# xcompact3d/x3d2

Measured on AMD Instinct MI355X. Metric: DoF*steps/s (whole node), TGV 512^3 per GPU, full fractional step, higher is better.
Workload: dtype f64; 1 GPU; TGV 512x512x512 all-periodic, Re=1600, dt=1e-3, RK3 (3 substeps/step), compact6/classic schemes, rocFFT Poisson (configs[2]); per_gpu=512^3, driver=fused, parallelism=domain decomposition 1x1x1, decomposition=yslabs, decomposition_requested=auto, poisson_z_first=228

## Files before the change

### include/x3d2_hip.h

```cpp
#ifndef X3D2_HIP_H
#define X3D2_HIP_H

#include <stddef.h>

#ifdef X3D_SINGLE_PREC
typedef float x3d_real;
#else
typedef double x3d_real;
#endif

#ifdef __cplusplus
extern "C" {
#endif

enum { X3D_DIR_X = 1, X3D_DIR_Y = 2, X3D_DIR_Z = 3, X3D_DIR_C = 4 };
enum { X3D_BC_PERIODIC = 0, X3D_BC_NEUMANN = 1, X3D_BC_DIRICHLET = 2, X3D_BC_HALO = -1 };
enum { X3D_X_FACE = 1100, X3D_Y_FACE = 1010, X3D_Z_FACE = 110 };
#define X3D_N_HALO 4

typedef struct x3d_backend x3d_backend;
typedef struct x3d_tdsops x3d_tdsops;
typedef struct x3d_poisson x3d_poisson;

const char *x3d_last_error(void);
// ... 188 lines not shown
                       const x3d_real *az, const x3d_real *bz);
int x3d_poisson_destroy(x3d_poisson *p);
int x3d_poisson_fft_forward(x3d_poisson *p, const x3d_real *f_in);
int x3d_poisson_postprocess_000(x3d_poisson *p);
int x3d_poisson_fft_backward(x3d_poisson *p, x3d_real *f_out);
int x3d_poisson_solve_000(x3d_poisson *p, x3d_real *f);
int x3d_poisson_enforce_periodicity_y(x3d_poisson *p, x3d_real *f_out, const x3d_real *f_in);
int x3d_poisson_undo_periodicity_y(x3d_poisson *p, x3d_real *f_out, const x3d_real *f_in);
int x3d_poisson_set_stretching(x3d_poisson *p, int sym, const x3d_real *a0, const x3d_real *a1);
int x3d_poisson_postprocess_010(x3d_poisson *p);
int x3d_poisson_solve_010(x3d_poisson *p, x3d_real *f, x3d_real *temp);
int x3d_poisson_solve_010_rows(x3d_poisson *p, x3d_real *f);
int x3d_transpose_xy(x3d_backend *b_src, x3d_backend *b_dst, x3d_real *dst, const x3d_real *src, int nx, int ny, int nz);
int x3d_transpose_xyz_zxy(x3d_backend *b_src, x3d_backend *b_dst, x3d_real *dst, const x3d_real *src, int nx, int ny, int nz);
int x3d_transpose_zxy_xyz(x3d_backend *b_src, x3d_backend *b_dst, x3d_real *dst, const x3d_real *src, int nx, int ny, int nz);
int x3d_poisson_enforce_periodicity_z(x3d_poisson *p, x3d_real *f_out, const x3d_real *f_in);
int x3d_poisson_undo_periodicity_z(x3d_poisson *p, x3d_real *f_out, const x3d_real *f_in);
int x3d_poisson_postprocess_011(x3d_poisson *p);
int x3d_poisson_get_spectral(x3d_poisson *p, x3d_real *host_interleaved);
int x3d_poisson_set_spectral(x3d_poisson *p, const x3d_real *host_interleaved);

typedef struct x3d_sfft x3d_sfft;
int x3d_sfft_create(x3d_backend *b, x3d_sfft **out, const int nglob[3], int pz, int rz);
int x3d_sfft_destroy(x3d_sfft *p);
int x3d_sfft_sizes(const x3d_sfft *p, long out[4]);
int x3d_sfft_set_waves(x3d_sfft *p, const x3d_real *waves, const x3d_real *ax, const x3d_real *bx, const x3d_real *ay,
                       const x3d_real *by, const x3d_real *az, const x3d_real *bz);
int x3d_sfft_forward_local(x3d_sfft *p, const x3d_real *f_in, x3d_real *sendbuf);
int x3d_sfft_fft_z(x3d_sfft *p, x3d_real *recvbuf, int dir);
int x3d_sfft_postprocess_000(x3d_sfft *p, x3d_real *recvbuf);
int x3d_sfft_backward_local(x3d_sfft *p, const x3d_real *recvbuf, x3d_real *f_out);
int x3d_sfft_create_parts(x3d_backend *b, x3d_sfft **out, const int nglob[3], int pz, int rz, int parts);
int x3d_sfft_fft_z_part(x3d_sfft *p, x3d_real *recvbuf, int dir, int part);
int x3d_sfft_postprocess_000_part(x3d_sfft *p, x3d_real *recvbuf, int part);

typedef struct x3d_sfft010 x3d_sfft010;
int x3d_sfft010_create(x3d_backend *b, x3d_sfft010 **out, const int nglob_cell[3], int pz, int rz);
int x3d_sfft010_destroy(x3d_sfft010 *p);
int x3d_sfft010_sizes(const x3d_sfft010 *p, long out[6]);
int x3d_sfft010_create_parts(x3d_backend *b, x3d_sfft010 **out, const int nglob_cell[3], int pz, int rz, int parts);
int x3d_sfft010_fft_z_part(x3d_sfft010 *p, x3d_real *recvbuf, int dir, int part);
int x3d_sfft010_postprocess_010_part(x3d_sfft010 *p, x3d_real *recvbuf, int part);
int x3d_sfft010_set_waves(x3d_sfft010 *p, const x3d_real *waves, const x3d_real *ax, const x3d_real *bx, const x3d_real *ay,
                          const x3d_real *by, const x3d_real *az, const x3d_real *bz);
int x3d_sfft010_set_stretching(x3d_sfft010 *p, int sym, const x3d_real *a0, const x3d_real *a1);
int x3d_sfft010_periodicity_y(x3d_sfft010 *p, x3d_real *f_out, const x3d_real *f_in, int undo);
int x3d_sfft010_forward_local(x3d_sfft010 *p, const x3d_real *f_in, x3d_real *sendbuf);
int x3d_sfft010_fft_z(x3d_sfft010 *p, x3d_real *recvbuf, int dir);
int x3d_sfft010_postprocess_010(x3d_sfft010 *p, x3d_real *recvbuf);
int x3d_sfft010_backward_local(x3d_sfft010 *p, const x3d_real *sendbuf, x3d_real *f_out);

int x3d_poisson_zfirst_ok(x3d_poisson *p, int *ok);
int x3d_tds_pair_zfirst_ok(x3d_backend *b, const x3d_tdsops *ta, const x3d_tdsops *tb, int *ok);
int x3d_poisson_zfirst_middle(x3d_poisson *p);
int x3d_poisson_zfirst_forward(x3d_poisson *p, const x3d_real *f_in);
int x3d_poisson_zfirst_backward(x3d_poisson *p, x3d_real *f_out);
int x3d_poisson_solve_000_zfirst(x3d_poisson *p, x3d_real *f);
int x3d_poisson_set_stretching_zfirst(x3d_poisson *p, int sym, const x3d_real *a0, const x3d_real *a1);
int x3d_poisson_create_proxy(x3d_backend *b, x3d_poisson **out, x3d_real *spectrum, int ny, long px, int (*middle)(void *user),
                             void *user);
int x3d_poisson_solve_010_rows_zfirst(x3d_poisson *p, x3d_real *f);
int x3d_tds_pair_zfirst(x3d_backend *b, x3d_poisson *poisson, int mode, x3d_real *out1, x3d_real *out2, const x3d_real *in1,
                        const x3d_real *in2, const x3d_tdsops *ta, const x3d_tdsops *tb, int *done);

typedef struct x3d_sfftz x3d_sfftz;
int x3d_sfftz_create(x3d_backend *b, x3d_sfftz **out, const int nglob_cell[3], int py, int ry, int parts);
int x3d_sfftz_destroy(x3d_sfftz *p);
int x3d_sfftz_sizes(const x3d_sfftz *p, long out[16]);
int x3d_sfftz_spectrum(const x3d_sfftz *p, x3d_real **c, int *ny, long *px);
int x3d_sfftz_set_waves(x3d_sfftz *p, const x3d_real *rw, const x3d_real *ax, const x3d_real *bx, const x3d_real *ay,
                        const x3d_real *by, const x3d_real *az, const x3d_real *bz);
int x3d_sfftz_tds_pair(x3d_sfftz *p, int mode, x3d_real *out1, x3d_real *out2, const x3d_real *in1, const x3d_real *in2,
                       const x3d_tdsops *ta, const x3d_tdsops *tb, int *done);
int x3d_sfftz_z(x3d_sfftz *p, x3d_real *f, int inverse);
int x3d_sfftz_z_field(x3d_sfftz *p, x3d_real *f, int inverse);
int x3d_sfftz_x_forward(x3d_sfftz *p, x3d_real *sendbuf, int part);
int x3d_sfftz_y_stage(x3d_sfftz *p, x3d_real *recvbuf, int part, int what);
int x3d_sfftz_x_backward(x3d_sfftz *p, const x3d_real *buf, int part);
int x3d_sfftz_tds_pair_rows(x3d_sfftz *p, int mode, x3d_real *out1, x3d_real *out2, const x3d_real *in1, const x3d_real *in2,
                            const x3d_tdsops *ta, const x3d_tdsops *tb, int y0, int nyr, int *done);
int x3d_sfftz_z_rows(x3d_sfftz *p, x3d_real *f, int inverse, int y0, int nyr);
int x3d_sfftz_x_forward_rows(x3d_sfftz *p, x3d_real *sendbuf, int part, int y0, int nyr);
int x3d_sfftz_x_backward_rows(x3d_sfftz *p, const x3d_real *buf, int part, int y0, int nyr);

typedef struct x3d_pfft x3d_pfft;
int x3d_pfft_create(x3d_backend *b, x3d_pfft **out, const int nglob_cell[3], int py, int pz, int ry, int rz);
int x3d_pfft_destroy(x3d_pfft *p);
int x3d_pfft_sizes(const x3d_pfft *p, long out[8]);
int x3d_pfft_set_waves(x3d_pfft *p, const x3d_real *waves_re, const x3d_real *ax, const x3d_real *bx,
                       const x3d_real *ay, const x3d_real *by, const x3d_real *az, const x3d_real *bz);
int x3d_pfft_fwd_x(x3d_pfft *p, const x3d_real *f_in);
int x3d_pfft_bwd_x(x3d_pfft *p, x3d_real *f_out);
int x3d_pfft_fft_y(x3d_pfft *p, int inverse);
int x3d_pfft_fft_z(x3d_pfft *p, int inverse);
int x3d_pfft_pack_xy(x3d_pfft *p, x3d_real *sendbuf);
int x3d_pfft_unpack_xy(x3d_pfft *p, const x3d_real *recvbuf);
int x3d_pfft_pack_yx(x3d_pfft *p, x3d_real *sendbuf);
int x3d_pfft_unpack_yx(x3d_pfft *p, const x3d_real *recvbuf);
int x3d_pfft_pack_yz(x3d_pfft *p, x3d_real *sendbuf);
int x3d_pfft_unpack_yz(x3d_pfft *p, const x3d_real *recvbuf);
int x3d_pfft_pack_zy(x3d_pfft *p, x3d_real *sendbuf);
int x3d_pfft_unpack_zy(x3d_pfft *p, const x3d_real *recvbuf);
int x3d_pfft_transpose_local(x3d_pfft *p, int which);
int x3d_pfft_own_chunk(x3d_pfft *p, const x3d_real *sendbuf, int rank);
int x3d_pfft_postprocess_000(x3d_pfft *p);
int x3d_pfft_create_parts(x3d_backend *b, x3d_pfft **out, const int nglob_cell[3], int py, int pz, int ry, int rz,
// ... 63 lines not shown
```

### x3d2_amd/_lib.py

```python
import ctypes
import os
import subprocess

from .common import X3dError

HERE = os.path.dirname(os.path.abspath(__file__))
SINGLE = os.environ.get("X3D_SINGLE_PREC") == "1"
LIB_PATH = os.path.join(HERE, "libx3d2_hip_sp.so" if SINGLE else "libx3d2_hip.so")
CSRC = os.path.join(HERE, "csrc")

REAL = ctypes.c_float if SINGLE else ctypes.c_double
NP_REAL = "float32" if SINGLE else "float64"
c_double_p = ctypes.POINTER(REAL)
c_int_p = ctypes.POINTER(ctypes.c_int)
VP = ctypes.c_void_p
I, D, SZT = ctypes.c_int, REAL, ctypes.c_size_t


def torch_real():
    import torch
    return torch.float32 if SINGLE else torch.float64

PROTOTYPES = {
    "x3d_last_error": (ctypes.c_char_p, []),
# ... 103 lines not shown
    "x3d_field_set_face_from_field": (I, [VP, VP, VP, c_int_p, D, I, D]),
    "x3d_set_field_data": (I, [VP, VP, c_double_p, c_int_p]),
    "x3d_get_field_data": (I, [VP, c_double_p, VP, c_int_p]),
    "x3d_set_field_data_pitched": (I, [VP, VP, c_double_p, I, I, c_int_p]),
    "x3d_get_field_data_pitched": (I, [VP, c_double_p, VP, I, I, c_int_p]),
    "x3d_poisson_create": (I, [VP, ctypes.POINTER(VP), c_int_p] + [c_double_p] * 7),
    "x3d_poisson_destroy": (I, [VP]),
    "x3d_poisson_fft_forward": (I, [VP, VP]),
    "x3d_poisson_postprocess_000": (I, [VP]),
    "x3d_poisson_fft_backward": (I, [VP, VP]),
    "x3d_poisson_solve_000": (I, [VP, VP]),
    "x3d_poisson_enforce_periodicity_y": (I, [VP, VP, VP]),
    "x3d_poisson_undo_periodicity_y": (I, [VP, VP, VP]),
    "x3d_poisson_set_stretching": (I, [VP, ctypes.c_int, c_double_p, c_double_p]),
    "x3d_sfftz_spectrum": (I, [VP, ctypes.POINTER(VP), c_int_p, ctypes.POINTER(ctypes.c_long)]),
    "x3d_poisson_create_proxy": (I, [VP, ctypes.POINTER(VP), VP, I, ctypes.c_long, VP, VP]),
    "x3d_poisson_set_stretching_zfirst": (I, [VP, ctypes.c_int, c_double_p, c_double_p]),
    "x3d_poisson_postprocess_010": (I, [VP]),
    "x3d_poisson_solve_010": (I, [VP, VP, VP]),
    "x3d_poisson_solve_010_rows": (I, [VP, VP]),
    "x3d_poisson_solve_010_rows_zfirst": (I, [VP, VP]),
    "x3d_poisson_get_spectral": (I, [VP, c_double_p]),
    "x3d_poisson_set_spectral": (I, [VP, c_double_p]),
    "x3d_sfft_create": (I, [VP, ctypes.POINTER(VP), c_int_p, I, I]),
    "x3d_sfft_create_parts": (I, [VP, ctypes.POINTER(VP), c_int_p, I, I, I]),
    "x3d_sfft_fft_z_part": (I, [VP, VP, I, I]),
    "x3d_sfft_postprocess_000_part": (I, [VP, VP, I]),
    "x3d_sfft_destroy": (I, [VP]),
    "x3d_sfft_sizes": (I, [VP, ctypes.POINTER(ctypes.c_long)]),
    "x3d_sfft_set_waves": (I, [VP] + [c_double_p] * 7),
    "x3d_sfft_forward_local": (I, [VP, VP, VP]),
    "x3d_sfft_fft_z": (I, [VP, VP, I]),
    "x3d_sfft_postprocess_000": (I, [VP, VP]),
    "x3d_sfft_backward_local": (I, [VP, VP, VP]),
    "x3d_sfft010_create": (I, [VP, ctypes.POINTER(VP), c_int_p, I, I]),
    "x3d_sfft010_create_parts": (I, [VP, ctypes.POINTER(VP), c_int_p, I, I, I]),
    "x3d_sfft010_fft_z_part": (I, [VP, VP, I, I]),
    "x3d_sfft010_postprocess_010_part": (I, [VP, VP, I]),
    "x3d_sfft010_destroy": (I, [VP]),
    "x3d_sfft010_sizes": (I, [VP, ctypes.POINTER(ctypes.c_long)]),
    "x3d_sfft010_set_waves": (I, [VP] + [c_double_p] * 7),
    "x3d_sfft010_set_stretching": (I, [VP, I, c_double_p, c_double_p]),
    "x3d_sfft010_periodicity_y": (I, [VP, VP, VP, I]),
    "x3d_sfft010_forward_local": (I, [VP, VP, VP]),
    "x3d_sfft010_fft_z": (I, [VP, VP, I]),
    "x3d_sfft010_postprocess_010": (I, [VP, VP]),
    "x3d_sfft010_backward_local": (I, [VP, VP, VP]),
    "x3d_poisson_zfirst_ok": (I, [VP, c_int_p]),
    "x3d_poisson_zfirst_middle": (I, [VP]),
    "x3d_poisson_zfirst_forward": (I, [VP, VP]),
    "x3d_poisson_zfirst_backward": (I, [VP, VP]),
    "x3d_poisson_solve_000_zfirst": (I, [VP, VP]),
    "x3d_tds_pair_zfirst": (I, [VP, VP, I, VP, VP, VP, VP, VP, VP, c_int_p]),
    "x3d_sfftz_create": (I, [VP, ctypes.POINTER(VP), c_int_p, I, I, I]),
    "x3d_sfftz_destroy": (I, [VP]),
    "x3d_sfftz_sizes": (I, [VP, ctypes.POINTER(ctypes.c_long)]),
    "x3d_sfftz_set_waves": (I, [VP] + [c_double_p] * 7),
    "x3d_sfftz_tds_pair": (I, [VP, I, VP, VP, VP, VP, VP, VP, c_int_p]),
    "x3d_sfftz_z": (I, [VP, VP, I]),
    "x3d_sfftz_z_field": (I, [VP, VP, I]),
    "x3d_sfftz_x_forward": (I, [VP, VP, I]),
    "x3d_sfftz_y_stage": (I, [VP, VP, I, I]),
    "x3d_sfftz_x_backward": (I, [VP, VP, I]),
    "x3d_sfftz_tds_pair_rows": (I, [VP, I, VP, VP, VP, VP, VP, VP, I, I, c_int_p]),
    "x3d_sfftz_z_rows": (I, [VP, VP, I, I, I]),
    "x3d_sfftz_x_forward_rows": (I, [VP, VP, I, I, I]),
    "x3d_sfftz_x_backward_rows": (I, [VP, VP, I, I, I]),
    "x3d_pfft_create": (I, [VP, ctypes.POINTER(VP), c_int_p, I, I, I, I]),
    "x3d_pfft_destroy": (I, [VP]),
    "x3d_pfft_sizes": (I, [VP, ctypes.POINTER(ctypes.c_long)]),
    "x3d_pfft_set_waves": (I, [VP] + [c_double_p] * 7),
    "x3d_pfft_fwd_x": (I, [VP, VP]),
    "x3d_pfft_bwd_x": (I, [VP, VP]),
    "x3d_pfft_fft_y": (I, [VP, I]),
    "x3d_pfft_fft_z": (I, [VP, I]),
    "x3d_pfft_pack_xy": (I, [VP, VP]),
    "x3d_pfft_unpack_xy": (I, [VP, VP]),
    "x3d_pfft_pack_yx": (I, [VP, VP]),
    "x3d_pfft_unpack_yx": (I, [VP, VP]),
    "x3d_pfft_pack_yz": (I, [VP, VP]),
    "x3d_pfft_unpack_yz": (I, [VP, VP]),
    "x3d_pfft_pack_zy": (I, [VP, VP]),
    "x3d_pfft_unpack_zy": (I, [VP, VP]),
    "x3d_pfft_transpose_local": (I, [VP, I]),
    "x3d_pfft_own_chunk": (I, [VP, VP, I]),
    "x3d_pfft_postprocess_000": (I, [VP]),
    "x3d_pfft_create_parts": (I, [VP, ctypes.POINTER(VP), c_int_p, I, I, I, I, I]),
    "x3d_pfft_part_layout": (I, [VP, ctypes.POINTER(ctypes.c_long)]),
    "x3d_pfft_fwd_a_part": (I, [VP, VP, VP, I]),
    "x3d_pfft_fwd_b_part": (I, [VP, VP, VP, I]),
    "x3d_pfft_fwd_c_part": (I, [VP, VP, I]),
    "x3d_pfft_bwd_c_part": (I, [VP, VP, I]),
    "x3d_pfft_bwd_b_part": (I, [VP, VP, VP, I]),
    "x3d_pfft_bwd_a_part": (I, [VP, VP, VP, I]),
    "x3d_stats_update_uvw": (I, [VP, VP, VP, VP, ctypes.POINTER(VP), D]),
    "x3d_stats_update_scalar": (I, [VP, VP, VP, VP, D]),
    "x3d_stats_derive": (I, [VP, ctypes.POINTER(VP), ctypes.POINTER(VP)]),
    "x3d_stats_profile_sums": (I, [VP, VP, VP, VP, c_int_p, I, VP]),
    "x3d_stats_profile_accumulate": (I, [VP, VP, VP, ctypes.c_long, D, D]),
    "x3d_ibm_create": (I, [VP, c_double_p, c_int_p, ctypes.POINTER(VP)]),
    "x3d_ibm_destroy": (I, [VP]),
    "x3d_ibm_counts": (I, [VP, ctypes.POINTER(ctypes.c_long)]),
    "x3d_ibm_body": (I, [VP, VP, VP, VP, VP, c_int_p]),
    "x3d_outflow_params": (I, [VP, VP, c_int_p, D, D, ctypes.POINTER(VP)]),
    "x3d_outflow_params_get": (I, [VP, c_double_p]),
    "x3d_cylinder_apply_bc": (I, [VP, VP, VP, VP, VP, VP, VP, c_int_p, VP]),
# ... 51 lines not shown
```

### x3d2_amd/csrc/backend.hip

```cpp
#include <mutex>

#include <algorithm>
#include <vector>

#include "common.h"

#include <unordered_map>
#include <unordered_set>

#include <cmath>

static thread_local char g_err[512] = "";

void x3d_set_error(const char *fmt, ...)
{
    va_list ap;
    va_start(ap, fmt);
    vsnprintf(g_err, sizeof g_err, fmt, ap);
    va_end(ap);
}

extern "C" const char *x3d_last_error(void) { return g_err; }
extern "C" int x3d_abi_version(void) { return 1; }
extern "C" int x3d_real_bytes(void) { return (int)sizeof(real_t); }
// ... 50 lines not shown
    X3D_HIP(hipMalloc(&b->red_buf, sizeof(real_t) * 2 * b->red_cap));
    X3D_HIP(hipHostMalloc(&b->red_host, sizeof(real_t) * 2 * b->red_cap));
    X3D_HIP(hipMalloc(&b->epi_dev, 512));
    b->lds_optin = new std::unordered_set<const void *>();
    X3D_HIP(hipEventCreate(&b->ev0));
    X3D_HIP(hipEventCreate(&b->ev1));
    *out = b;
    return 0;
}

extern "C" int x3d_backend_create_like(x3d_backend **out, const x3d_backend *like, const int dims_vert[3])
{
    X3D_RANGE(__func__);
    X3D_REQUIRE(like, "x3d_backend_create_like: null argument");
    return x3d_backend_create(out, dims_vert, like->device, (void *)like->stream);
}

extern "C" int x3d_backend_destroy(x3d_backend *b)
{
    X3D_RANGE(__func__);
    if (!b) return 0;
    if (b->ipc_maps) {
        auto *v = static_cast<std::vector<void *> *>(b->ipc_maps);
        for (void *p : *v) (void)hipIpcCloseMemHandle(p);
        delete v;
    }
    hipFree(b->send_s); hipFree(b->send_e);
    hipFree(b->scratch[0]); hipFree(b->scratch[1]); hipFree(b->scratch[2]);
    x3d_prof_enable_c(b, 0);
    hipFree(b->red_buf); hipHostFree(b->red_host); hipFree(b->epi_dev);
    if (b->stats_part) hipFree(b->stats_part);
    if (b->bc_params) hipFree(b->bc_params);
    if (b->bc_part) hipFree(b->bc_part);
    hipEventDestroy(b->ev0); hipEventDestroy(b->ev1);
    delete static_cast<std::unordered_set<const void *> *>(b->lds_optin);
    x3d_lazy_destroy(b);
    delete b;
    return 0;
}

int x3d_lds_optin(x3d_backend *b, const void *kernel)
{
    auto *seen = static_cast<std::unordered_set<const void *> *>(b->lds_optin);
    if (seen->count(kernel)) return 0;
    X3D_HIP(hipFuncSetAttribute(kernel, hipFuncAttributeMaxDynamicSharedMemorySize, 160 * 1024));
    seen->insert(kernel);
    return 0;
}

extern "C" long x3d_backend_counter(const x3d_backend *b, int which)
{
    X3D_RANGE(__func__);
    if (!b) return -1;
    return which == 0 ? b->n_tq3 : (which == 1 ? b->n_upd : (which == 2 ? b->n_halo : (which == 3 ? b->n_sync : -1)));
}

extern "C" int x3d_backend_set_stream(x3d_backend *b, void *stream)
{
    X3D_RANGE(__func__);
    X3D_REQUIRE(b, "null backend");
    b->stream = (hipStream_t)stream;
    return 0;
}

extern "C" int x3d_backend_set_comm_reserve(x3d_backend *b, int ncus)
{
    X3D_RANGE(__func__);
    X3D_REQUIRE(b, "null backend");
    X3D_REQUIRE(ncus >= 0 && ncus < X3D_NCU / 2, "x3d_backend_set_comm_reserve: 0 .. %d CUs", X3D_NCU / 2 - 1);
    b->comm_reserve = ncus;
    return 0;
}

extern "C" int x3d_backend_set_ring(x3d_backend *b, int dir, int periodic_over_all_ranks)
{
    X3D_RANGE(__func__);
    X3D_REQUIRE(b && x3d_dir_ok(dir), "x3d_backend_set_ring: null backend or bad direction");
    b->ring[dir] = periodic_over_all_ranks ? 1 : 0;
    return 0;
}

extern "C" size_t x3d_block_elems(const x3d_backend *b) { return b ? b->nblock : 0; }

extern "C" int x3d_padded_dims(const x3d_backend *b, int d[3])
{
    X3D_RANGE(__func__);
    X3D_REQUIRE(b && d, "null argument");
    d[0] = b->nxp; d[1] = b->nyp; d[2] = b->nzp;
    return 0;
}

extern "C" int x3d_device_sync(x3d_backend *b)
{
    X3D_RANGE(__func__);
    if (b) X3D_LAZY_FLUSH(b);
    X3D_LAZY_EAGER(b);
    X3D_REQUIRE(b, "null backend");
    X3D_HIP(hipStreamSynchronize(b->stream));
    return 0;
}

static std::unordered_map<real_t *, void *> g_block_base;
static int g_block_count = 0;
static std::mutex g_block_mutex;

extern "C" int x3d_block_alloc(x3d_backend *b, real_t **out)
{
// ... 840 lines not shown
```

### x3d2_amd/csrc/common.h

```cpp
#pragma once
#include <hip/hip_runtime.h>

#include <cstdarg>
#include <cstdio>
#include <cstring>
#include <vector>

#include "../../include/x3d2_hip.h"

typedef x3d_real real_t;
#ifdef X3D_SINGLE_PREC
typedef float2 real2_t;
#define make_real2 make_float2
#else
typedef double2 real2_t;
#define make_real2 make_double2
#endif
#ifdef X3D_SINGLE_PREC
#define X3D_FFT_R2C HIPFFT_R2C
#define X3D_FFT_C2R HIPFFT_C2R
#define X3D_FFT_C2C HIPFFT_C2C
#define x3d_fftExecR2C hipfftExecR2C
#define x3d_fftExecC2R hipfftExecC2R
#define x3d_fftExecC2C hipfftExecC2C
// ... 43 lines not shown
    __builtin_amdgcn_wave_barrier();
    __builtin_amdgcn_fence(__ATOMIC_ACQUIRE, "wavefront");
}

typedef real_t x3d_d2v __attribute__((ext_vector_type(2)));
__device__ __forceinline__ real2_t ldg_stream(const real2_t *p)
{
    const x3d_d2v v = __builtin_nontemporal_load(reinterpret_cast<const x3d_d2v *>(p));
    return make_real2(v.x, v.y);
}
__device__ __forceinline__ void stg_stream(real2_t *p, real2_t v)
{
    const x3d_d2v w = {v.x, v.y};
    __builtin_nontemporal_store(w, reinterpret_cast<x3d_d2v *>(p));
}

static __device__ __attribute__((used)) float g_vmcnt_sink[32 * 1024];
template <int N>
__device__ __forceinline__ void vmcnt_pad_stores()
{
#pragma unroll
    for (int k = 0; k < N; k++) __builtin_nontemporal_store(0.0f, &g_vmcnt_sink[k * 1024 + (threadIdx.x & 1023)]);
}

__host__ __device__ static inline unsigned long long x3d_mix64(unsigned long long z)
{
    z += 0x9E3779B97F4A7C15ull;
    z = (z ^ (z >> 30)) * 0xBF58476D1CE4E5B9ull;
    z = (z ^ (z >> 27)) * 0x94D049BB133111EBull;
    return z ^ (z >> 31);
}

struct PencilGeom {
    int np;
    int dim0;
    long s0, s1, rs;
};

struct x3d_backend {
    int device;
    hipStream_t stream;
    int nx, ny, nz;
    int ring[4];
    int nxp, nyp, nzp;
    size_t nblock;
    real_t *send_s, *send_e;
    real_t *scratch[3];
    real_t *red_buf;
    real_t *red_host;
    int red_cap;
    long n_upd;
    long n_tq3;
    long n_halo;
    void *epi_dev;
    hipEvent_t ev0, ev1;
    void *ipc_maps;
    struct x3d_prof *prof;
    unsigned prof_mask;
    int pair_yperm;
    void *lds_optin;
    struct x3d_lazy *lazy;
    int comm_reserve;
    double *stats_part;
    long stats_cap;
    real_t *bc_params;
    double *bc_part;
    long n_sync;
};
#define X3D_BC_PARTS 1024
struct TileEpi {
    real_t *y;
    const real_t *base;
    const real_t *x[5];
    real_t c[5];
    int n, ipend, store;
};
#define X3D_NCU 256
static inline int x3d_persistent_blocks(const x3d_backend *b, long want)
{
    const long cap = X3D_NCU - (b->comm_reserve > 0 && b->comm_reserve < X3D_NCU / 2 ? b->comm_reserve : 0);
    return (int)(want > cap ? cap : want);
}

bool x3d_lazy_active(const x3d_backend *b);
void x3d_lazy_destroy(x3d_backend *b);
void x3d_lazy_register(x3d_backend *b, real_t *h);
void x3d_lazy_unregister(x3d_backend *b, real_t *h);
int x3d_lazy_flush_c(x3d_backend *b);
int x3d_lazy_sync_c(x3d_backend *b);
int x3d_lazy_in(x3d_backend *b, const real_t *h, const real_t **out);
int x3d_lazy_out(x3d_backend *b, real_t *h, bool full, real_t **out);
int x3d_lazy_transeq(x3d_backend *b, int dir, real_t *du, real_t *dv, real_t *dw, const real_t *u, const real_t *v,
                     const real_t *w, real_t nu, const x3d_tdsops *t0, const x3d_tdsops *t1, const x3d_tdsops *t2,
                     const x3d_tdsops *t3);
int x3d_lazy_tds(x3d_backend *b, real_t *du, const real_t *u, const x3d_tdsops *t, int dir);
int x3d_lazy_species(x3d_backend *b, int dir, real_t *dspec, const real_t *uvw, const real_t *spec, real_t nu,
                     const x3d_tdsops *t0, const x3d_tdsops *t1, const x3d_tdsops *t2, int accumulate);
int x3d_lazy_copy(x3d_backend *b, real_t *dst, const real_t *src);
int x3d_lazy_sum(x3d_backend *b, real_t *u, const real_t *u_, int dir);
int x3d_lazy_vecadd(x3d_backend *b, real_t a, const real_t *x, real_t bb, real_t *y);
int x3d_lazy_unary(x3d_backend *b, int kind, real_t *f, const real_t *x, real_t a);
int x3d_lazy_fft(x3d_backend *b, int which, void *poisson, real_t *f);
int x3d_lazy_setface(x3d_backend *b, real_t *f, const real_t *f_start, const int dims[3]);
bool x3d_lazy_set_executing(x3d_backend *b, bool on);
struct LazyScope {
    x3d_backend *b;
// ... 140 lines not shown
```

### x3d2_amd/csrc/sfftz.hip

```cpp
#include "zfft_tile.h"

#define SZ_PX 520
#define SZ_MAXPARTS 8

int x3d_fft512_init();
const real2_t *x3d_fft512_twiddles();
int x3d_fft512_peers_yl(x3d_backend *b, real2_t *R, long W, int npeers, const real_t *rw, const real_t *ab, int nx, int ny,
                        int nz, int xs, int xoff, int kz0, int part);
int x3d_ztile_fft_run(x3d_backend *b, real_t *f, const ZfArg &zf, bool fwd, int y0, int nyr);
int x3d_ytile_tds_pair_zf(x3d_backend *b, int mode, real_t *out1, real_t *out2, const real_t *in1, const real_t *in2,
                          const x3d_tdsops *ta, const x3d_tdsops *tb, const ZfArg &zf, bool *done, int y0, int nyr);

struct x3d_sfftz {
    x3d_backend *b;
    int py, ry, xs, xoff, parts;
    int kz0[SZ_MAXPARTS + 1];
    long off[SZ_MAXPARTS + 1];
    real2_t *c;
    real_t *rw;
    real_t *ab;
};

template <bool PACK>
__global__ void __launch_bounds__(512)
// ... 79 lines not shown
    return 0;
}

extern "C" int x3d_sfftz_set_waves(x3d_sfftz *p, const real_t *rw, const real_t *ax, const real_t *bx, const real_t *ay,
                                   const real_t *by, const real_t *az, const real_t *bz)
{
    X3D_RANGE(__func__);
    X3D_REQUIRE(p && rw && ax && bx && ay && by && az && bz, "null argument");
    X3D_HIP(hipMemcpy(p->rw, rw, sizeof(real_t) * 257 * p->xs * 512 * p->py, hipMemcpyHostToDevice));
    real_t *d = p->ab;
    const real_t *src[6] = {ax, bx, ay, by, az, bz};
    const int len[6] = {512, 512, 512 * p->py, 512 * p->py, 512, 512};
    for (int i = 0; i < 6; i++) {
        X3D_HIP(hipMemcpy(d, src[i], sizeof(real_t) * len[i], hipMemcpyHostToDevice));
        d += len[i];
    }
    return 0;
}

static ZfArg zfarg(const x3d_sfftz *p) { return ZfArg{p->c, x3d_fft512_twiddles(), 512, (long)SZ_PX}; }

extern "C" int x3d_sfftz_tds_pair(x3d_sfftz *p, int mode, real_t *out1, real_t *out2, const real_t *in1, const real_t *in2,
                                  const x3d_tdsops *ta, const x3d_tdsops *tb, int *done)
{
    X3D_RANGE(__func__);
    X3D_REQUIRE(p && ta && tb && done, "x3d_sfftz_tds_pair: null argument");
    X3D_REQUIRE(mode == 0 || mode == 1, "x3d_sfftz_tds_pair: mode must be 0 or 1");
    X3D_REQUIRE(mode == 0 ? (in1 && in2) : (out1 && out2 && out1 != out2), "x3d_sfftz_tds_pair: null argument");
    X3D_LAZY_SYNC(p->b);
    X3D_LAZY_EAGER(p->b);
    bool ok = false;
    *done = 0;
    if (int rc = x3d_ytile_tds_pair_zf(p->b, mode, out1, out2, in1, in2, ta, tb, zfarg(p), &ok, 0, -1)) return rc;
    *done = ok ? 1 : 0;
    return 0;
}
extern "C" int x3d_sfftz_tds_pair_rows(x3d_sfftz *p, int mode, real_t *out1, real_t *out2, const real_t *in1,
                                       const real_t *in2, const x3d_tdsops *ta, const x3d_tdsops *tb, int y0, int nyr, int *done)
{
    X3D_RANGE(__func__);
    X3D_REQUIRE(p && ta && tb && done, "x3d_sfftz_tds_pair_rows: null argument");
    X3D_REQUIRE(mode == 0 || mode == 1, "x3d_sfftz_tds_pair_rows: mode must be 0 or 1");
    X3D_REQUIRE(mode == 0 ? (in1 && in2) : (out1 && out2 && out1 != out2), "x3d_sfftz_tds_pair_rows: null argument");
    X3D_REQUIRE(y0 >= 0 && nyr >= 0 && y0 + nyr <= 512, "x3d_sfftz_tds_pair_rows: rows [%d, %d) of 512", y0, y0 + nyr);
    X3D_LAZY_SYNC(p->b);
    X3D_LAZY_EAGER(p->b);
    bool ok = false;
    *done = 0;
    if (int rc = x3d_ytile_tds_pair_zf(p->b, mode, out1, out2, in1, in2, ta, tb, zfarg(p), &ok, y0, nyr)) return rc;
    *done = ok ? 1 : 0;
    return 0;
}

extern "C" int x3d_sfftz_z(x3d_sfftz *p, real_t *f, int inverse)
{
    X3D_RANGE(__func__);
    X3D_REQUIRE(p && f, "null argument");
    X3D_LAZY_SYNC(p->b);
    return x3d_ztile_fft_run(p->b, f, zfarg(p), !inverse, 0, -1);
}
extern "C" int x3d_sfftz_z_field(x3d_sfftz *p, real_t *f, int inverse)
{
    X3D_RANGE(__func__);
    X3D_REQUIRE(p && f, "null argument");
    if (inverse) { X3D_LAZY_OUT(p->b, f, true); }
    else {
        const real_t *fi = f;
        X3D_LAZY_IN(p->b, fi);
        f = const_cast<real_t *>(fi);
    }
    return x3d_ztile_fft_run(p->b, f, zfarg(p), !inverse, 0, -1);
}
extern "C" int x3d_sfftz_z_rows(x3d_sfftz *p, real_t *f, int inverse, int y0, int nyr)
{
    X3D_RANGE(__func__);
    X3D_REQUIRE(p && f, "null argument");
    X3D_REQUIRE(y0 >= 0 && nyr >= 0 && y0 + nyr <= 512, "x3d_sfftz_z_rows: rows [%d, %d) of 512", y0, y0 + nyr);
    X3D_LAZY_SYNC(p->b);
    return x3d_ztile_fft_run(p->b, f, zfarg(p), !inverse, y0, nyr);
}

#define SZ_PART(p, m, name) X3D_REQUIRE((p) && (m) >= 0 && (m) < (p)->parts, name ": part %d of %d", (m), (p) ? (p)->parts : 0)

template <bool PACK>
static int x_xchg(x3d_sfftz *p, real_t *buf, int m, int y0 = 0, int nyr = 512)
{
    const int lds = sizeof(real2_t) * (8 * FP + 256);
    X3D_LDS_OPTIN(p->b, (k_c2c512_x_xchg<PACK>));
    const int kzc = p->kz0[m + 1] - p->kz0[m];
    if (nyr == 0) return 0;
    long blocks = ((long)kzc * nyr + 7) / 8;
    if (blocks > 2048) blocks = 2048;
    ProfScope ps(p->b, X3D_K_FFT, PACK ? 1 : 2);
    hipLaunchKernelGGL((k_c2c512_x_xchg<PACK>), dim3((unsigned)blocks), dim3(512), lds, p->b->stream, p->c,
                       (real2_t *)buf + p->off[m], x3d_fft512_twiddles(), p->kz0[m], kzc, p->xs, y0, nyr);
    X3D_HIP(hipGetLastError());
    return 0;
}
extern "C" int x3d_sfftz_x_forward(x3d_sfftz *p, real_t *sendbuf, int m)
{
    X3D_RANGE(__func__);
    SZ_PART(p, m, "x3d_sfftz_x_forward");
    X3D_REQUIRE(sendbuf, "null argument");
    return x_xchg<true>(p, sendbuf, m);
}
extern "C" int x3d_sfftz_y_stage(x3d_sfftz *p, real_t *recvbuf, int m, int what)
// ... 37 lines not shown
```

### x3d2_amd/csrc/xscan.hip

```cpp
#include "common.h"


int npmax_of(const x3d_backend *b);

#include "xscan_core.h"
#include "zfft_tile.h"


template <bool ACC>
__device__ __forceinline__ void store_rows_q8(real_t *__restrict__ orow, int lane, const real_t (&r)[8],
                                              real_t scale)
{
    const int j = lane & 3;
    real_t a0 = r[0], a1 = r[1], b0 = r[2], b1 = r[3], c0 = r[4], c1 = r[5], d0 = r[6], d1 = r[7];
    rotl_pairs(a0, a1, b0, b1, c0, c1, d0, d1, j);
    b0 = dpp_quad(b0, 1); b1 = dpp_quad(b1, 1);
    c0 = dpp_quad(c0, 2); c1 = dpp_quad(c1, 2);
    d0 = dpp_quad(d0, 3); d1 = dpp_quad(d1, 3);
    rotl_pairs(a0, a1, b0, b1, c0, c1, d0, d1, j);
    real2_t *__restrict__ o2 = reinterpret_cast<real2_t *>(orow + (lane & ~3) * 8) + j;
    real2_t v0, v1, v2, v3;
    if (ACC) {
        v0 = o2[0]; v1 = o2[4]; v2 = o2[8]; v3 = o2[12];
        v0.x += scale * a0; v0.y += scale * a1;
// ... 1558 lines not shown
        return t->tab.bulk_only && t->n_tds == 64 * Q && t->tab.n_rhs == t->n_tds;
    };
    if (!fast(ta) || !fast(tb) || (dir == X3D_DIR_Y ? b->ny : b->nz) != 64 * Q || b->nx % 16 != 0) return 0;
    if (dir == X3D_DIR_Z) { const char *e = getenv("X3D_NO_ZTILE"); if (e && e[0] == '1') return 0; }
    const bool narrow = stencil_narrow(ta) && stencil_narrow(tb);
    static int uni_on = -1;
    if (uni_on < 0) { const char *e = getenv("X3D_NO_UNIFORM"); uni_on = (e && e[0] == '1') ? 0 : 1; }
    const bool uni = uni_on && ta->uniform && tb->uniform;
    const bool circ = narrow && uni && circ_env_on() && (halo ? pair_halo_circ(b, dir, ta, tb) : (ta->circ_ok && tb->circ_ok));
    const size_t lds = sizeof(real_t) * ((size_t)(circ ? 0 : (mode == 2 ? 1 : 2) * LT_N(Q) * 64) + 16 * (64 * Q + 4) + (halo ? 128 + 64 : 0));
    if (lds > 160 * 1024) return 0;
    const long pxy = (long)b->nxp * b->nyp;
    const int ntx = b->nx / 16;
    int tile0, ntiles;
    tile_range(b, dir, other0, nother, ntx, &tile0, &ntiles);
    const int permn = b->pair_yperm;
    if (permn > 0 && (dir != X3D_DIR_Z || mode == 2 || tile0 != 0 || (ntiles > 0 && ntiles != ntx * b->ny))) return 0;
    if (ntiles <= 0) { *done = true; return 0; }
    const long rstride = dir == X3D_DIR_Y ? (long)b->nxp : pxy, ostride = dir == X3D_DIR_Y ? pxy : (long)b->nxp;
    if (128 * rstride * X3D_RB >= (1L << 32)) return 0;
    const int blocks = x3d_persistent_blocks(b, ntiles);
    const TileHalo th = halo ? *halo : TileHalo{nullptr, nullptr, 0, 0, 0, 0, 0};
    ProfScope ps(b, X3D_K_TDS_FWD, dir);
#define GO(Q_, M_, N_, H_, U_, C_)                                                                              \
    do {                                                                                                        \
        X3D_LDS_OPTIN(b, (k_ytile_tds_pair<Q_, M_, N_, H_, false, U_, C_, false>));                             \
        hipLaunchKernelGGL((k_ytile_tds_pair<Q_, M_, N_, H_, false, U_, C_, false>), dim3(blocks), dim3(1024), lds, b->stream, out1, out2, \
                           in1, in2, xop_of(ta), xop_of(tb), ntx, tile0, ntiles, rstride, ostride, th, permn,   \
                           ZfArg{}, ta->circ, tb->circ);                                                        \
    } while (0)
#define GOH(Q_, M_, N_, U_) do { if (halo) GO(Q_, M_, N_, true, U_, false); else GO(Q_, M_, N_, false, U_, false); } while (0)
#define GON(Q_, M_) do { if (circ && halo) GO(Q_, M_, true, true, true, true); else if (circ) GO(Q_, M_, true, false, true, true); else if (narrow && uni) GOH(Q_, M_, true, true); else if (narrow) GOH(Q_, M_, true, false); else GOH(Q_, M_, false, false); } while (0)
#define GOM(Q_) do { if (mode == 0) GON(Q_, 0); else if (mode == 1) GON(Q_, 1); else GON(Q_, 2); } while (0)
    if (Q == 8) GOM(8); else GOM(4);
#undef GOM
#undef GON
#undef GOH
#undef GO
    if (halo) b->n_halo++;
    X3D_HIP(hipGetLastError());
    *done = true;
    return 0;
}

bool x3d_zfirst_pairs_ok(const x3d_backend *b, const x3d_tdsops *ta, const x3d_tdsops *tb)
{
    if (!use_ytile() || !xscan_ok(ta) || !xscan_ok(tb) || ta->tab.Q != 8 || tb->tab.Q != 8) return false;
    auto fast = [&](const x3d_tdsops *t) { return t->tab.bulk_only && t->n_tds == 512 && t->tab.n_rhs == t->n_tds; };
    if (!fast(ta) || !fast(tb) || b->nz != 512 || b->nx % 16 != 0) return false;
    if (sizeof(real_t) * ((size_t)2 * LT_NC(8) * 64 + ZF_AREA_DOUBLES + 512) > 160 * 1024) return false;
    return 128 * (long)b->nxp * b->nyp * X3D_RB < (1L << 32);
}

int x3d_ytile_tds_pair_zf(x3d_backend *b, int mode, real_t *out1, real_t *out2, const real_t *in1, const real_t *in2,
                          const x3d_tdsops *ta, const x3d_tdsops *tb, const ZfArg &zf, bool *done, int y0, int nyr)
{
    *done = false;
    if (mode < 0 || mode > 1 || zf.ny > b->ny || (zf.permn == 0 && zf.ny != b->ny) || !x3d_zfirst_pairs_ok(b, ta, tb)) return 0;
    if (nyr < 0) { y0 = 0; nyr = zf.ny; }
    X3D_REQUIRE(y0 >= 0 && nyr >= 0 && y0 + nyr <= zf.ny, "tds_pair (z-first): rows [%d, %d) of %d", y0, y0 + nyr, zf.ny);
    X3D_REQUIRE(zf.permn == 0 || (zf.permn == zf.ny && y0 == 0 && nyr == zf.ny), "tds_pair (z-first): interleaved rows, whole blocks only");
    if (nyr == 0) { *done = true; return 0; }
    const bool narrow = stencil_narrow(ta) && stencil_narrow(tb);
    static int uni_on = -1;
    if (uni_on < 0) { const char *e = getenv("X3D_NO_UNIFORM"); uni_on = (e && e[0] == '1') ? 0 : 1; }
    const bool uni = uni_on && ta->uniform && tb->uniform;
    const bool circ = narrow && uni && circ_env_on() && ta->circ_ok && tb->circ_ok;
    const size_t lds = sizeof(real_t) * ((size_t)(circ ? 0 : 2 * LT_NC(8) * 64) + ZF_AREA_DOUBLES + 512);
    const long pxy = (long)b->nxp * b->nyp;
    const int ntx = b->nx / 16, ntiles = ntx * nyr, tile0 = ntx * y0;
    const int blocks = x3d_persistent_blocks(b, ntiles);
    const TileHalo th{nullptr, nullptr, 0, 0, 0, 0, 0};
    ProfScope ps(b, X3D_K_TDS_FWD, X3D_DIR_Z);
#define GOD(M_, N_, U_, C_, D_)                                                                                 \
    do {                                                                                                        \
        X3D_LDS_OPTIN(b, (k_ytile_tds_pair<8, M_, N_, false, true, U_, C_, D_>));                               \
        hipLaunchKernelGGL((k_ytile_tds_pair<8, M_, N_, false, true, U_, C_, D_>), dim3(blocks), dim3(1024), lds, b->stream, out1, \
                           out2, in1, in2, xop_of(ta), xop_of(tb), ntx, tile0, ntiles, pxy, (long)b->nxp, th, 0, zf, ta->circ, tb->circ); \
    } while (0)
#define GO(M_, N_, U_, C_) GOD(M_, N_, U_, C_, (C_) && (M_) == 1)
#define GOU(M_) do { if (circ) GO(M_, true, true, true); else if (narrow && uni) GO(M_, true, true, false); else if (narrow) GO(M_, true, false, false); else GO(M_, false, false, false); } while (0)
    if (mode == 0) GOU(0); else GOU(1);
#undef GOU
#undef GO
#undef GOD
    X3D_HIP(hipGetLastError());
    *done = true;
    return 0;
}

int x3d_tds_halo_fix(x3d_backend *b, int dir, int mode, real_t *out1, real_t *out2, const real_t *brecv,
                     const x3d_tdsops *ta, const x3d_tdsops *tb)
{
    const PencilGeom g = x3d_geom(b, dir);
    const bool hc = pair_halo_circ(b, dir, ta, mode == 2 ? ta : tb);
    const TdsTab &tta = hc ? ta->tabc : ta->tab, &ttb = hc ? tb->tabc : tb->tab;
    const int wsa = hc ? ta->halo_ws_c : ta->halo_ws, wsb = hc ? tb->halo_ws_c : tb->halo_ws;
    const int wea = hc ? ta->halo_we_c : ta->halo_we, web = hc ? tb->halo_we_c : tb->halo_we;
    const int ws = mode == 2 ? wsa : (wsa > wsb ? wsa : wsb);
    const int we = mode == 2 ? wea : (wea > web ? wea : web);
    dim3 grid((g.np + 255) / 256, ws + we >= ta->n_tds ? 1 : 2);
    const int ws1 = grid.y == 1 ? ta->n_tds : ws;
    const int permn = b->pair_yperm;
    X3D_REQUIRE(permn == 0 || (dir == X3D_DIR_Z && mode != 2), "tds_halo_fix: interleaved rows are for z pairs");
    ProfScope ps(b, X3D_K_TDS_BWD, dir);
    if (mode == 0) hipLaunchKernelGGL(k_tds_halo_fix<0>, grid, dim3(256), 0, b->stream, out1, out2, brecv, tta, ttb, g, ws1, we, permn);
    else if (mode == 1) hipLaunchKernelGGL(k_tds_halo_fix<1>, grid, dim3(256), 0, b->stream, out1, out2, brecv, tta, ttb, g, ws1, we, permn);
    else hipLaunchKernelGGL(k_tds_halo_fix<2>, grid, dim3(256), 0, b->stream, out1, out2, brecv, tta, tta, g, ws1, we, 0);
    X3D_HIP(hipGetLastError());
    return 0;
}

int x3d_transeq_halo_fix_launch(x3d_backend *b, int dir, real_t *const r[3], const real_t *conv, real_t nu,
                                const real_t *brecv, const x3d_tdsops *der1st, const x3d_tdsops *der2nd)
{
    const PencilGeom g = x3d_geom(b, dir);
    const bool hc = transeq_halo_circ(b, dir, der1st, der2nd);
    const TdsTab &tt1 = hc ? der1st->tabc : der1st->tab, &tt2 = hc ? der2nd->tabc : der2nd->tab;
    const int ws1_ = hc ? der1st->halo_ws_c : der1st->halo_ws, ws2_ = hc ? der2nd->halo_ws_c : der2nd->halo_ws;
    const int we1_ = hc ? der1st->halo_we_c : der1st->halo_we, we2_ = hc ? der2nd->halo_we_c : der2nd->halo_we;
    const int ws = ws1_ > ws2_ ? ws1_ : ws2_;
    const int we = we1_ > we2_ ? we1_ : we2_;
    dim3 grid((g.np + 255) / 256, ws + we >= der1st->n_tds ? 1 : 2);
    const int ws1 = grid.y == 1 ? der1st->n_tds : ws;
    ProfScope ps(b, X3D_K_TRANSEQ_BWD, dir);
    hipLaunchKernelGGL(k_transeq_halo_fix, grid, dim3(256), 0, b->stream, r[0], r[1], r[2], conv, brecv, tt1,
// ... 231 lines not shown
```

Before: 3.174 billion DoF*steps/s.

## Add 512-thread z-first tridiagonal-pair kernel with fused z-FFT for circulant ops

Adds a new k_zfpair2 kernel for the z-first Poisson path, used by default in FP64 when the circulant, uniform, narrow-stencil case applies. It runs 512-thread blocks with a two-blocks-per-CU persistent cap and uses only the area and twiddle shared memory, dropping the large tile buffer the old 1024-thread kernel needed. It fuses both circulant solves with the 512-point z FFT and the real/complex split, and prefetches the next tile's input in half-chunks. The aim is higher occupancy and less shared-memory and sync cost per tile, at the price of a new, more intricate code path with its own index mapping. A test entry point and a launch counter are also added.

```diff
diff --git a/include/x3d2_hip.h b/include/x3d2_hip.h
--- a/include/x3d2_hip.h
+++ b/include/x3d2_hip.h
@@ -264,6 +264,9 @@
 
 int x3d_poisson_zfirst_ok(x3d_poisson *p, int *ok);
 int x3d_tds_pair_zfirst_ok(x3d_backend *b, const x3d_tdsops *ta, const x3d_tdsops *tb, int *ok);
+int x3d_tds_pair_zfirst_at(x3d_backend *b, x3d_real *spectrum, int ny, long px, int permn, int mode, x3d_real *out1,
+                           x3d_real *out2, const x3d_real *in1, const x3d_real *in2, const x3d_tdsops *ta,
+                           const x3d_tdsops *tb, int y0, int nyr, int *done);
 int x3d_poisson_zfirst_middle(x3d_poisson *p);
 int x3d_poisson_zfirst_forward(x3d_poisson *p, const x3d_real *f_in);
 int x3d_poisson_zfirst_backward(x3d_poisson *p, x3d_real *f_out);
diff --git a/x3d2_amd/_lib.py b/x3d2_amd/_lib.py
--- a/x3d2_amd/_lib.py
+++ b/x3d2_amd/_lib.py
@@ -179,6 +179,7 @@
     "x3d_poisson_zfirst_backward": (I, [VP, VP]),
     "x3d_poisson_solve_000_zfirst": (I, [VP, VP]),
     "x3d_tds_pair_zfirst": (I, [VP, VP, I, VP, VP, VP, VP, VP, VP, c_int_p]),
+    "x3d_tds_pair_zfirst_at": (I, [VP, VP, I, ctypes.c_long, I, I, VP, VP, VP, VP, VP, VP, I, I, c_int_p]),
     "x3d_sfftz_create": (I, [VP, ctypes.POINTER(VP), c_int_p, I, I, I]),
     "x3d_sfftz_destroy": (I, [VP]),
     "x3d_sfftz_sizes": (I, [VP, ctypes.POINTER(ctypes.c_long)]),
diff --git a/x3d2_amd/csrc/backend.hip b/x3d2_amd/csrc/backend.hip
--- a/x3d2_amd/csrc/backend.hip
+++ b/x3d2_amd/csrc/backend.hip
@@ -126,7 +126,7 @@
 {
     X3D_RANGE(__func__);
     if (!b) return -1;
-    return which == 0 ? b->n_tq3 : (which == 1 ? b->n_upd : (which == 2 ? b->n_halo : (which == 3 ? b->n_sync : -1)));
+    return which == 0 ? b->n_tq3 : (which == 1 ? b->n_upd : (which == 2 ? b->n_halo : (which == 3 ? b->n_sync : (which == 4 ? b->n_zfpair2 : -1))));
 }
 
 extern "C" int x3d_backend_set_stream(x3d_backend *b, void *stream)
diff --git a/x3d2_amd/csrc/common.h b/x3d2_amd/csrc/common.h
--- a/x3d2_amd/csrc/common.h
+++ b/x3d2_amd/csrc/common.h
@@ -119,6 +119,7 @@
     long n_upd;
     long n_tq3;
     long n_halo;
+    long n_zfpair2;
     void *epi_dev;
     hipEvent_t ev0, ev1;
     void *ipc_maps;
diff --git a/x3d2_amd/csrc/sfftz.hip b/x3d2_amd/csrc/sfftz.hip
--- a/x3d2_amd/csrc/sfftz.hip
+++ b/x3d2_amd/csrc/sfftz.hip
@@ -155,6 +155,27 @@
     return 0;
 }
 
+extern "C" int x3d_tds_pair_zfirst_at(x3d_backend *b, real_t *spectrum, int ny, long px, int permn, int mode, real_t *out1,
+                                      real_t *out2, const real_t *in1, const real_t *in2, const x3d_tdsops *ta,
+                                      const x3d_tdsops *tb, int y0, int nyr, int *done)
+{
+    X3D_RANGE(__func__);
+    X3D_REQUIRE(b && spectrum && ta && tb && done, "x3d_tds_pair_zfirst_at: null argument");
+    X3D_REQUIRE(mode == 0 || mode == 1, "x3d_tds_pair_zfirst_at: mode must be 0 or 1");
+    X3D_REQUIRE(mode == 0 ? (in1 && in2) : (out1 && out2 && out1 != out2), "x3d_tds_pair_zfirst_at: null argument");
+    X3D_REQUIRE(ny > 0 && ny <= b->ny && px >= b->nx && px % 16 == 0 && (permn == 0 || permn == ny),
+                "x3d_tds_pair_zfirst_at: a spectrum of %d rows of %ld (block: %d rows of %d)", ny, px, b->ny, b->nx);
+    X3D_LAZY_SYNC(b);
+    X3D_LAZY_EAGER(b);
+    if (int rc = x3d_fft512_init()) return rc;
+    bool ok = false;
+    *done = 0;
+    const ZfArg zf{reinterpret_cast<real2_t *>(spectrum), x3d_fft512_twiddles(), ny, px, permn};
+    if (int rc = x3d_ytile_tds_pair_zf(b, mode, out1, out2, in1, in2, ta, tb, zf, &ok, y0, nyr)) return rc;
+    *done = ok ? 1 : 0;
+    return 0;
+}
+
 extern "C" int x3d_sfftz_z(x3d_sfftz *p, real_t *f, int inverse)
 {
     X3D_RANGE(__func__);
diff --git a/x3d2_amd/csrc/xscan.hip b/x3d2_amd/csrc/xscan.hip
--- a/x3d2_amd/csrc/xscan.hip
+++ b/x3d2_amd/csrc/xscan.hip
@@ -1634,6 +1634,8 @@
     return 128 * (long)b->nxp * b->nyp * X3D_RB < (1L << 32);
 }
 
+int x3d_zfpair2_launch(x3d_backend *b, int mode, real_t *out1, real_t *out2, const real_t *in1, const real_t *in2,
+                       const CircOp &ca, const CircOp &cb, int ntx, int tile0, int ntiles, const ZfArg &zf);
 int x3d_ytile_tds_pair_zf(x3d_backend *b, int mode, real_t *out1, real_t *out2, const real_t *in1, const real_t *in2,
                           const x3d_tdsops *ta, const x3d_tdsops *tb, const ZfArg &zf, bool *done, int y0, int nyr)
 {
@@ -1654,6 +1656,15 @@
     const int blocks = x3d_persistent_blocks(b, ntiles);
     const TileHalo th{nullptr, nullptr, 0, 0, 0, 0, 0};
     ProfScope ps(b, X3D_K_TDS_FWD, X3D_DIR_Z);
+#ifndef X3D_SINGLE_PREC
+    static int zf2_on = -1;
+    if (zf2_on < 0) { const char *e = getenv("X3D_NO_ZFPAIR2"); zf2_on = (e && e[0] == '1') ? 0 : 1; }
+    if (circ && zf2_on) {
+        if (int rc = x3d_zfpair2_launch(b, mode, out1, out2, in1, in2, ta->circ, tb->circ, ntx, tile0, ntiles, zf)) return rc;
+        *done = true;
+        return 0;
+    }
+#endif
 #define GOD(M_, N_, U_, C_, D_)                                                                                 \
     do {                                                                                                        \
         X3D_LDS_OPTIN(b, (k_ytile_tds_pair<8, M_, N_, false, true, U_, C_, D_>));                               \
diff --git a/x3d2_amd/csrc/zfpair2.hip b/x3d2_amd/csrc/zfpair2.hip
--- /dev/null
+++ b/x3d2_amd/csrc/zfpair2.hip
@@ -0,0 +1,242 @@
+#include "xscan_core.h"
+#include "zfft_tile.h"
+
+#ifndef X3D_SINGLE_PREC
+
+__device__ __forceinline__ int zp_slot(int r, int w) { return (((r >> 3) + w) & 63) * 9 + (r & 7); }
+__device__ __forceinline__ const real2_t *zp_row(const real_t *base, long prow, int i, unsigned voff)
+{
+    return reinterpret_cast<const real2_t *>(reinterpret_cast<const char *>(base + (long)(64 * i) * prow) + voff);
+}
+struct ZpRows { real2_t v0, v1, v2, v3, v4, v5, v6, v7; };
+struct ZpHalf { real2_t v0, v1, v2, v3; };
+struct ZpRest { real2_t v4, v5, v6, v7, v8; };
+struct ZpModes { real2_t v0, v1, v2, v3, v4, v5, v6, v7, v8; };
+#define ZP_EACH8(X) X(0) X(1) X(2) X(3) X(4) X(5) X(6) X(7)
+#ifndef X3D_ZFPAIR2_PFE0
+#define X3D_ZFPAIR2_PFE0 false
+#endif
+#ifndef X3D_ZFPAIR2_PFE1
+#define X3D_ZFPAIR2_PFE1 false
+#endif
+
+template <int MODE, bool PFE>
+__global__ void __launch_bounds__(512, 4)
+    k_zfpair2(real_t *out1, real_t *out2, const real_t *__restrict__ in1, const real_t *__restrict__ in2, int ntx, int tile0,
+              int ntiles, long prow, long pplane, ZfArg zf, CircOp ca, CircOp cb)
+{
+    extern __shared__ real_t lt[];
+    constexpr int Q = 8, NI = 8;
+    real2_t *area = reinterpret_cast<real2_t *>(lt);
+    real2_t *tws = area + ZF_AREA_DOUBLES / 2;
+    if (threadIdx.x < 256) tws[threadIdx.x] = zf.tw[threadIdx.x];
+    const long kzs = (long)zf.ny * zf.px;
+    auto zf_row = [&](int tl) {
+        int r = tl / ntx;
+        if (zf.permn > 0 && r < zf.permn) r = (r & 1) ? zf.permn - ((r + 1) >> 1) : (r >> 1);
+        return zf.c + (long)r * zf.px + (long)(tl % ntx) * 16;
+    };
+    ntiles += tile0;
+    int lane = threadIdx.x & 63;
+    const int wave = __builtin_amdgcn_readfirstlane(threadIdx.x >> 6);
+    real2_t *pen = area + wave * ZF_PEN;
+    const int cy = threadIdx.x >> 3;
+    int cc = threadIdx.x & 7;
+    const unsigned voff = (unsigned)(((long)cy * prow + 2 * cc) * X3D_RB);
+    auto cslot = [&](int i) { return cc * ZF_PEN + ((wave + 8 * i + cc) & 63) * 9 + (cy & 7); };
+    auto gload = [&](const real_t *__restrict__ src) {
+        ZpRows v;
+#define X(i) v.v##i = *zp_row(src, prow, i, voff);
+        ZP_EACH8(X)
+#undef X
+        return v;
+    };
+    auto gload4 = [&](const real_t *__restrict__ src, int h) {
+        ZpHalf v;
+        v.v0 = *zp_row(src, prow, 4 * h, voff); v.v1 = *zp_row(src, prow, 4 * h + 1, voff);
+        v.v2 = *zp_row(src, prow, 4 * h + 2, voff); v.v3 = *zp_row(src, prow, 4 * h + 3, voff);
+        return v;
+    };
+    auto to_tile4 = [&](const ZpHalf &v, int h) {
+        area[cslot(4 * h)] = v.v0; area[cslot(4 * h + 1)] = v.v1; area[cslot(4 * h + 2)] = v.v2; area[cslot(4 * h + 3)] = v.v3;
+    };
+    auto to_tile = [&](const ZpRows &v) {
+#define X(i) area[cslot(i)] = v.v##i;
+        ZP_EACH8(X)
+#undef X
+    };
+    auto from_tile = [&](real_t *o) {
+#pragma unroll
+        for (int i = 0; i < NI; i++) *const_cast<real2_t *>(zp_row(o, prow, i, voff)) = area[cslot(i)];
+    };
+    auto pick = [&](V2 (&b)[Q]) {
+        const real2_t *src = pen + ((lane + wave) & 63) * 9;
+#pragma unroll
+        for (int q = 0; q < Q; q++) {
+            const real2_t t2_ = src[q];
+            b[q] = V2{t2_.x, t2_.y};
+        }
+    };
+    auto put = [&](const V2 (&r)[Q]) {
+        real2_t *dst = pen + ((lane + wave) & 63) * 9;
+#pragma unroll
+        for (int q = 0; q < Q; q++) dst[q] = make_real2(r[q].a, r[q].b);
+    };
+    auto tile_off = [&](int tl) { return (long)(tl / ntx) * pplane + (long)(tl % ntx) * 16; };
+    const int mr = threadIdx.x >> 4, mx = threadIdx.x & 15, t2s = zf_t2(mr, mx);
+    const unsigned moff = (unsigned)(((long)mr * kzs + mx) * (long)sizeof(real2_t));
+    auto mode_row = [&](const real2_t *crow, int i) {
+        return reinterpret_cast<const real2_t *>(reinterpret_cast<const char *>(crow + (long)(32 * i) * kzs) + moff);
+    };
+    auto mload = [&](const real2_t *__restrict__ crow) {
+        ZpHalf v;
+        v.v0 = *mode_row(crow, 0); v.v1 = *mode_row(crow, 1); v.v2 = *mode_row(crow, 2); v.v3 = *mode_row(crow, 3);
+        return v;
+    };
+    auto mload_rest = [&](const real2_t *__restrict__ crow) {
+        ZpRest v;
+        v.v4 = *mode_row(crow, 4); v.v5 = *mode_row(crow, 5); v.v6 = *mode_row(crow, 6); v.v7 = *mode_row(crow, 7);
+        v.v8 = *mode_row(crow, threadIdx.x < 16 ? 8 : 0);
+        return v;
+    };
+    __syncthreads();
+    ZpHalf nxt{};
+    ZpHalf spn{};
+    if (tile0 + (int)blockIdx.x < ntiles) {
+        if constexpr (MODE == 1) spn = mload(zf_row(tile0 + blockIdx.x));
+        else nxt = gload4(in1 + tile_off(tile0 + blockIdx.x), 0);
+    }
+    for (int tl = tile0 + blockIdx.x; tl < ntiles; tl += gridDim.x) {
+        const long off = tile_off(tl);
+        const int tn = tl + gridDim.x;
+        asm volatile("" : "+v"(lane), "+v"(cc));
+        V2 b[Q], w2[Q + 8], ra[Q], rb[Q];
+        real2_t a[8];
+        if constexpr (MODE == 0) {
+            const ZpHalf nx2 = gload4(in1 + off, 1);
+            const ZpRows g2 = gload(in2 + off);
+            to_tile4(nxt, 0);
+            to_tile4(nx2, 1);
+            __syncthreads();
+            pick(b);
+#pragma unroll
+            for (int q = 0; q < Q; q++) asm volatile("" : "+v"(b[q].a), "+v"(b[q].b));
+            __syncthreads();
+            window_from_body<Q, V2>(w2, b, lane);
+            circ_solve<Q, true, V2>(w2, ra, ca, lane);
+            to_tile(g2);
+            __syncthreads();
+            pick(b);
+            if (PFE && tn < ntiles) nxt = gload4(in1 + tile_off(tn), 0);
+            window_from_body<Q, V2>(w2, b, lane);
+            circ_solve<Q, true, V2>(w2, rb, cb, lane);
+#pragma unroll
+            for (int q = 0; q < Q; q++) ra[q] = V2{ra[q].a + 1.0 * rb[q].a, ra[q].b + 1.0 * rb[q].b};
+            wave_lds_fence();
+            put(ra);
+            wave_lds_fence();
+#pragma unroll
+            for (int k = 0; k < 8; k++) a[k] = pen[zp_slot(lane + 64 * k, wave)];
+            fft512_wave<-1>(a, pen, tws, lane);
+#pragma unroll
+            for (int k = 0; k < 8; k++) pen[lane + 64 * k] = a[k];
+            wave_lds_fence();
+            if (!PFE && tn < ntiles) nxt = gload4(in1 + tile_off(tn), 0);
+            real2_t A[5], B[5];
+#pragma unroll
+            for (int k = 0; k < 5; k++) {
+                const int idx = lane + 64 * k;
+                if (k < 4 || lane == 0) {
+                    const real2_t x = a[k], y = pen[(512 - idx) & 511];
+                    A[k] = make_real2(0.5 * (x.x + y.x), 0.5 * (x.y - y.y));
+                    B[k] = make_real2(0.5 * (x.y + y.y), -0.5 * (x.x - y.x));
+                }
+            }
+            __syncthreads();
+#pragma unroll
+            for (int k = 0; k < 5; k++) {
+                const int idx = lane + 64 * k;
+                if (k < 4 || lane == 0) {
+                    area[zf_t2(idx, 2 * wave)] = A[k];
+                    area[zf_t2(idx, 2 * wave + 1)] = B[k];
+                }
+            }
+            __syncthreads();
+            {
+                const real2_t *crow = zf_row(tl);
+#pragma unroll
+                for (int i = 0; i < 9; i++)
+                    if (i < 8 || threadIdx.x < 16) *const_cast<real2_t *>(mode_row(crow, i)) = area[t2s + 512 * i];
+            }
+            __syncthreads();
+        } else {
+            {
+                const ZpRest sr = mload_rest(zf_row(tl));
+                area[t2s] = spn.v0; area[t2s + 512] = spn.v1; area[t2s + 1024] = spn.v2; area[t2s + 1536] = spn.v3;
+                area[t2s + 2048] = sr.v4; area[t2s + 2560] = sr.v5; area[t2s + 3072] = sr.v6; area[t2s + 3584] = sr.v7;
+                if (threadIdx.x < 16) area[t2s + 4096] = sr.v8;
+            }
+            __syncthreads();
+#pragma unroll
+            for (int k = 0; k < 8; k++) {
+                const int m = lane + 64 * k, mm = m <= 256 ? m : 512 - m;
+                real2_t A = area[zf_t2(mm, 2 * wave)], B = area[zf_t2(mm, 2 * wave + 1)];
+                if (m > 256) { A.y = -A.y; B.y = -B.y; }
+                a[k] = make_real2(A.x - B.y, A.y + B.x);
+            }
+            __syncthreads();
+            fft512_wave<1>(a, pen, tws, lane);
+#pragma unroll
+            for (int k = 0; k < 8; k++) pen[zp_slot(lane + 64 * k, wave)] = a[k];
+            wave_lds_fence();
+            pick(b);
+            if (PFE && tn < ntiles) spn = mload(zf_row(tn));
+            window_from_body<Q, V2>(w2, b, lane);
+            circ_solve<Q, true, V2>(w2, ra, ca, lane);
+            wave_lds_fence();
+            put(ra);
+            __syncthreads();
+            from_tile(out1 + off);
+            asm volatile("" : "+v"(lane) : "v"(ra[0].a));
+            circ_solve<Q, true, V2>(w2, rb, cb, lane);
+            if (!PFE && tn < ntiles) spn = mload(zf_row(tn));
+            __syncthreads();
+            put(rb);
+            __syncthreads();
+            from_tile(out2 + off);
+            __syncthreads();
+        }
+    }
+}
+
+int x3d_zfpair2_launch(x3d_backend *b, int mode, real_t *out1, real_t *out2, const real_t *in1, const real_t *in2,
+                       const CircOp &ca, const CircOp &cb, int ntx, int tile0, int ntiles, const ZfArg &zf)
+{
+    const size_t lds = sizeof(real_t) * (ZF_AREA_DOUBLES + 512);
+    X3D_REQUIRE(32 * (long)zf.ny * zf.px * (long)sizeof(real2_t) < (1L << 32), "tds_pair (z-first): a spectrum of %d rows of %ld",
+                zf.ny, zf.px);
+    const long pxy = (long)b->nxp * b->nyp;
+    const int cap = 2 * x3d_persistent_blocks(b, X3D_NCU), blocks = ntiles < cap ? ntiles : cap;
+#define GO(M_, P_)                                                                                              \
+    do {                                                                                                        \
+        X3D_LDS_OPTIN(b, (k_zfpair2<M_, P_>));                                                                  \
+        hipLaunchKernelGGL((k_zfpair2<M_, P_>), dim3(blocks), dim3(512), lds, b->stream, out1, out2, in1, in2, ntx, tile0, \
+                           ntiles, pxy, (long)b->nxp, zf, ca, cb);                                              \
+    } while (0)
+    if (mode == 0) GO(0, X3D_ZFPAIR2_PFE0); else GO(1, X3D_ZFPAIR2_PFE1);
+#undef GO
+    X3D_HIP(hipGetLastError());
+    b->n_zfpair2++;
+    return 0;
+}
+
+#else
+
+int x3d_zfpair2_launch(x3d_backend *, int, real_t *, real_t *, const real_t *, const real_t *, const CircOp &, const CircOp &,
+                       int, int, int, const ZfArg &)
+{
+    x3d_set_error("x3d_zfpair2_launch: FP64 only");
+    return 2;
+}
+
+#endif
```

New measurement: 3.188 billion DoF*steps/s (median of 6 runs). No clear change (+0.4%).
